# ArchDD/CPP-Raytracer-Rasterizer

Measured on AMD Instinct MI355X. Metric: Mrays/s (primary+shadow), higher is better.
Workload: dtype f32

## Files before the change

cpp-raytracer-rasterizer_amd/csrc/rt_trace.hip:

```cpp
#include "rt_trace_frame.hpp"

#include <float.h>

namespace mirt {


__global__ __launch_bounds__(256) void k_geo_table(const float *__restrict__ tris15, int n, GeoRow *__restrict__ geo, ShadeRow *__restrict__ shade)
{
    const int t = blockIdx.x * blockDim.x + threadIdx.x;
    if (t >= n) return;
    const float *t15 = tris15 + (size_t)15 * t;
    const v3 v0 = ld3(t15), e1 = sub3(ld3(t15 + 3), v0), e2 = sub3(ld3(t15 + 6), v0);
    GeoRow g;
    g.g0 = make_float4(v0.x, v0.y, v0.z, e1.x);
    g.g1 = make_float4(e1.y, e1.z, e2.x, e2.y);
    g.g2 = make_float4(e2.z, 0.0f, 0.0f, 0.0f);
    geo[t] = g;
    const v3 nd = normalize3(ld3(t15 + 9));
    ShadeRow sr;
    sr.n = make_float4(nd.x, nd.y, nd.z, 0.0f);
    sr.col = make_float4(t15[12], t15[13], t15[14], 0.0f);
    shade[t] = sr;
}

__global__ __launch_bounds__(256) void k_expand_light_rows(const uint32_t *__restrict__ bin_off, const uint32_t *__restrict__ entries,
                                                           int nlights, uint32_t keys_per_light,
                                                           const OriginRow *__restrict__ light_tab, int n,
                                                           LightRow *__restrict__ rows, const uint32_t *__restrict__ pair_count, uint32_t pair_cap,
                                                           uint32_t *__restrict__ row_tri )
{
    if (pair_count && *pair_count > pair_cap) return;
    const uint32_t first = bin_off[0], total = bin_off[(size_t)nlights * keys_per_light];
    for (uint32_t p = first + blockIdx.x * blockDim.x + threadIdx.x; p < total; p += gridDim.x * blockDim.x) {
        int k = 0;
        while (k + 1 < nlights && bin_off[(size_t)(k + 1) * keys_per_light] <= p) k++;
        const uint32_t tri = entries[p];
        rows[p] = light_tab[(size_t)k * n + tri];
        if (row_tri) row_tri[p] = tri;
    }
}

#ifndef MIRT_TR_STAGE
#define MIRT_TR_STAGE 16
#endif
constexpr int TR_STAGE = MIRT_TR_STAGE;
constexpr int TR_DRAIN = 64;
constexpr int TR_QUEUE = 96;
constexpr int TR_PIX = 128;
static_assert(TR_STAGE == 16, "the staging lanes are split 16 / 16 between the two tiles");

struct TrWaveLds {
    union {
        struct {
            float4 rows[TR_STAGE * 6];
            float4 geo[TR_STAGE * 2 * 3];
        };
        struct {
            float4 ray[TR_PIX];
            uint8_t sink;
        };
    };
    float4 q[TR_QUEUE];
    unsigned long long best[TR_PIX];
    uint2 qa[TR_QUEUE];
    union {
        float px[TR_PIX];
        float thr[TR_PIX];
    };
    float py[TR_PIX], pz[TR_PIX];
    uint8_t flag[TR_PIX];
};
static_assert(sizeof(TrWaveLds) % 16 == 0, "per-wave LDS slice must keep 16-byte alignment");
static_assert(sizeof(TrWaveLds) == 8064, "20 waves share a CU's LDS: the ray table overlays the staging, it adds nothing");

__device__ __forceinline__ void wave_lds_fence()
{
    __builtin_amdgcn_fence(__ATOMIC_RELEASE, "wavefront");
    __builtin_amdgcn_wave_barrier();
    __builtin_amdgcn_fence(__ATOMIC_ACQUIRE, "wavefront");
}

template <bool SHADOW>
__device__ __forceinline__ void tr_drain(TrWaveLds &s, int lane, int count, const float4 *__restrict__ geo, v3 start,
                                         const uint32_t *__restrict__ row_tri = nullptr, bool lazy_geo = false)
{
    wave_lds_fence();
    if (lane < count) {
        const float4 e = s.q[lane];
        uint2 a = s.qa[lane];
        float t, u, v;
        div3_sel(e.w, e.y, e.z, e.x, __builtin_amdgcn_ballot_w64(exact_quotients_outside(e.w, e.y, e.z, e.x)), t, u, v);
        if (u + v <= 1.0f && u >= 0.0f && v >= 0.0f && t >= 0.0f) {
            float4 g0, g1, g2;
            if (SHADOW) {
                const uint32_t tri = row_tri ? row_tri[a.y] : a.y;
                const float4 *g = geo + (size_t)tri * 3;
                g0 = g[0]; g1 = g[1]; g2 = g[2];
            } else if (lazy_geo) {
                const float4 *g = geo + (size_t)a.y * 3;
                g0 = g[0]; g1 = g[1]; g2 = g[2];
                a.x &= 0xFFu;
            } else {
                const float4 *g = s.geo + (a.x >> 8) * 3;
                g0 = g[0]; g1 = g[1]; g2 = g[2];
                a.x &= 0xFFu;
            }
            const v3 v0 = V3(g0.x, g0.y, g0.z), e1 = V3(g0.w, g1.x, g1.y), e2 = V3(g1.z, g1.w, g2.x);
            const v3 p = add3(add3(v0, scale3(e1, u)), scale3(e2, v));
            const float dist = distance3(start, p);
            if (SHADOW) {
                if (dist < s.thr[a.x]) s.flag[a.x] = 1;
            } else {
                s.flag[a.x] = 1;
                const unsigned long long key = min_t_key(dist, (int)a.y);
                atomicMin(&s.best[a.x], key);
                __builtin_amdgcn_fence(__ATOMIC_ACQ_REL, "wavefront");
                if (s.best[a.x] == key) { s.px[a.x] = p.x; s.py[a.x] = p.y; s.pz[a.x] = p.z; }
            }
        }
    }
    wave_lds_fence();
}

template <bool SHADOW>
__device__ __forceinline__ void tr_drain_full(TrWaveLds &s, int lane, int &qn, const float4 *__restrict__ geo, v3 start,
                                              const uint32_t *__restrict__ row_tri = nullptr, bool lazy_geo = false)
{
    tr_drain<SHADOW>(s, lane, TR_DRAIN, geo, start, row_tri, lazy_geo);
    const int rest = qn - TR_DRAIN;
    float4 e = make_float4(0.0f, 0.0f, 0.0f, 0.0f);
    uint2 a = make_uint2(0u, 0u);
    if (lane < rest) { e = s.q[TR_DRAIN + lane]; a = s.qa[TR_DRAIN + lane]; }
    wave_lds_fence();
    if (lane < rest) { s.q[lane] = e; s.qa[lane] = a; }
    qn = rest;
    wave_lds_fence();
}

__device__ __forceinline__ unsigned long long wballot(bool p) { return __builtin_amdgcn_ballot_w64(p); }

__device__ __forceinline__ int wave_rank(unsigned long long m)
{
    return (int)__builtin_amdgcn_mbcnt_hi((uint32_t)(m >> 32), __builtin_amdgcn_mbcnt_lo((uint32_t)m, 0u));
}

__device__ __forceinline__ void cube_bin_of2(const v3p &rd, uint32_t face_base0, int cube_bins, uint32_t *bin0, uint32_t *bin1)
{
    f2 a, b, m;
    int face[2];
#pragma unroll
    for (int h = 0; h < 2; h++) {
        const float x = h ? rd.x.y : rd.x.x, y = h ? rd.y.y : rd.y.x, z = h ? rd.z.y : rd.z.x;
        const float ax = fabsf(x), ay = fabsf(y), az = fabsf(z);
        int k;
        float mm, aa, bb, sgn;
        if (ax >= ay && ax >= az) { k = 0; mm = ax; sgn = x; aa = y; bb = z; }
        else if (ay >= az) { k = 1; mm = ay; sgn = y; aa = z; bb = x; }
        else { k = 2; mm = az; sgn = z; aa = x; bb = y; }
        face[h] = 2 * k + (sgn < 0.0f ? 1 : 0);
        if (h) { a.y = aa; b.y = bb; m.y = mm; } else { a.x = aa; b.x = bb; m.x = mm; }
    }
    const f2 im = { __builtin_amdgcn_rcpf(m.x), __builtin_amdgcn_rcpf(m.y) };
    const f2 u = a * im, v = b * im;
    const float half = 0.5f * (float)cube_bins;
    const uint32_t per_face = (uint32_t)(cube_bins * cube_bins);
#pragma unroll
    for (int h = 0; h < 2; h++) {
        const float uu = h ? u.y : u.x, vv = h ? v.y : v.x;
        int i = (int)floorf((uu + 1.0f) * half);
        int j = (int)floorf((vv + 1.0f) * half);
        i = min(max(i, 0), cube_bins - 1);
        j = min(max(j, 0), cube_bins - 1);
        const uint32_t bin = face_base0 + (uint32_t)face[h] * per_face + (uint32_t)j * cube_bins + (uint32_t)i;
        if (h) *bin1 = bin; else *bin0 = bin;
    }
}

__device__ __forceinline__ uint32_t cube_bin_of1(v3 rd, uint32_t face_base0, int cube_bins)
{
    const float ax = fabsf(rd.x), ay = fabsf(rd.y), az = fabsf(rd.z);
    int k;
    float m, a, b, sgn;
    if (ax >= ay && ax >= az) { k = 0; m = ax; sgn = rd.x; a = rd.y; b = rd.z; }
    else if (ay >= az) { k = 1; m = ay; sgn = rd.y; a = rd.z; b = rd.x; }
    else { k = 2; m = az; sgn = rd.z; a = rd.x; b = rd.y; }
    const int face = 2 * k + (sgn < 0.0f ? 1 : 0);
    const float im = __builtin_amdgcn_rcpf(m);
    const float u = a * im, v = b * im, half = 0.5f * (float)cube_bins;
    int i = (int)floorf((u + 1.0f) * half);
    int j = (int)floorf((v + 1.0f) * half);
    i = min(max(i, 0), cube_bins - 1);
    j = min(max(j, 0), cube_bins - 1);
    return face_base0 + (uint32_t)face * (uint32_t)(cube_bins * cube_bins) + (uint32_t)j * cube_bins + (uint32_t)i;
}


__global__ __launch_bounds__(64) void k_tile_order(const uint32_t *__restrict__ cam_off, int cam_shells, int tiles_x, int j0, int j1,
                                                   uint32_t *__restrict__ counters, uint32_t pair_cap, TilePairRec *__restrict__ order, uint32_t seg)
{
    const int pairs_x = (tiles_x + 1) / 2, lane = threadIdx.x;
    const int ty = j0 + (int)blockIdx.y, px = (int)blockIdx.x * 64 + lane;
    const uint32_t group = ((uint32_t)ty >> ORDER_STRIPE_SHIFT) & (ORDER_GROUPS - 1);
    TilePairRec r = { 0u, 0u, 0u, 0u };
    int cls = -1;
    if (px < pairs_x) {
        const uint32_t tile = (uint32_t)(ty * tiles_x + 2 * px);
        r.txy = (uint32_t)(2 * px) | ((uint32_t)ty << 16);
        cls = 0;
        if (counters[0] <= pair_cap) {
            const uint32_t b0 = cam_off[(size_t)tile * cam_shells], b1 = cam_off[(size_t)(tile + 1) * cam_shells];
            r.beg = b0; r.nA = b1 - b0;
            r.nB = 2 * px + 1 < tiles_x ? cam_off[(size_t)(tile + 2) * cam_shells] - b1 : 0u;
            cls = (int)min(max(r.nA, r.nB) / ORDER_CLASS_STEP, (uint32_t)(ORDER_CLASSES - 1));
        }
    }
    unsigned long long m[ORDER_CLASSES];
    uint32_t mine = 0;
#pragma unroll
    for (int c = 0; c < ORDER_CLASSES; c++) {
        m[c] = __builtin_amdgcn_ballot_w64(cls == c);
        if (lane == c) mine = (uint32_t)__popcll(m[c]);
    }
    uint32_t base = 0;
    if (lane < ORDER_CLASSES && mine) base = atomicAdd(&counters[16 + group * ORDER_CLASSES + lane], mine);
#pragma unroll
    for (int c = 0; c < ORDER_CLASSES; c++) {
        const uint32_t bc = (uint32_t)__builtin_amdgcn_readlane((int)base, c);
        if (cls == c) order[((size_t)group * ORDER_CLASSES + c) * seg + bc + (uint32_t)__popcll(m[c] & ((1ull << lane) - 1ull))] = r;
    }
}

#ifndef MIRT_TR_WAVES
#define MIRT_TR_WAVES 4
#endif
#ifndef MIRT_TR_WAVES_MIN
#define MIRT_TR_WAVES_MIN 3
#endif
template <bool AA, bool STATS, int WAVES = MIRT_TR_WAVES>
__global__ __launch_bounds__(64 * TR_WG_WAVES) __attribute__((amdgpu_waves_per_eu(WAVES == 5 ? 5 : MIRT_TR_WAVES_MIN, WAVES))) void k_rt_trace2(const RtTraceFrame tf)
{
    extern __shared__ __attribute__((aligned(16))) float4 s_all[];
    const RtFrame &f = tf.f;
    static_assert(TR_WG_WAVES == 1, "the wave -> tile pair map below and the LDS slice assume one wave per workgroup");
    const int lane = threadIdx.x & 63;
    TrWaveLds &s = reinterpret_cast<TrWaveLds *>(s_all)[0];

    const uint32_t group = blockIdx.x & (ORDER_GROUPS - 1);
    const uint32_t w = blockIdx.x >> 3;
    const uint32_t flags = tf.flags;
    const uint4 *cp = reinterpret_cast<const uint4 *>(__builtin_assume_aligned(tf.order_count + group * ORDER_CLASSES, 32));
    const uint4 c0 = cp[0], c1 = cp[1];
    const uint32_t npairs = *tf.pair_count, nlpairs = *tf.light_pair_count, nsel = *tf.sel_count;
    const int W = f.W, H = f.H;
    TilePairRec rec;
    {
        const uint32_t cnt[ORDER_CLASSES] = { c0.x, c0.y, c0.z, c0.w, c1.x, c1.y, c1.z, c1.w };
        uint32_t sum = 0, first = 0;
        int cls = ORDER_CLASSES - 1;
#pragma unroll
        for (int c = ORDER_CLASSES - 1; c >= 0; c--) {
            sum += cnt[c];
            const bool past = w >= sum;
            first = past ? sum : first;
            cls = past ? c - 1 : cls;
        }
        if (cls < 0) return;
        const uint32_t at = w - first;
        const uint4 r4 = *reinterpret_cast<const uint4 *>(tf.order + ((size_t)group * ORDER_CLASSES + (uint32_t)cls) * tf.order_seg + at);
        rec.txy = r4.x; rec.beg = r4.y; rec.nA = r4.z; rec.nB = r4.w;
    }
    const int txA = (int)(rec.txy & 0xFFFFu), ty = (int)(rec.txy >> 16);
    const bool enB = txA + 1 < tf.tiles_x;
    const int xA = txA * BIN_TILE + (lane & 7), xB = xA + BIN_TILE, y = ty * BIN_TILE + (lane >> 3);
    const bool okY = y >= f.y0 && y < f.y1;
    const bool okA = okY && xA < W, okB = enB && okY && xB < W;
    const unsigned long long okmA = wballot(okA), okmB = wballot(okB);
    const unsigned nokA = (unsigned)__popcll(okmA), nokB = (unsigned)__popcll(okmB);
#ifdef MIRT_TR_TIMING
    const long long tm0 = __builtin_amdgcn_s_memtime();
    long long tm_last = tm0, tm_seg[10] = { 0, 0, 0, 0, 0, 0, 0, 0, 0, 0 };
#define TM_SEG(i) { const long long now_ = __builtin_amdgcn_s_memtime(); tm_seg[i] += now_ - tm_last; tm_last = now_; }
#else
#define TM_SEG(i)
#endif
    const bool brute = npairs > tf.pair_cap;
    const bool brute_l = nlpairs > tf.light_pair_cap;
    const v3 cam = ld3(f.cam);
    const int rs = AA ? f.aa : 1;

    const uint32_t begA = rec.beg, begB = rec.beg + rec.nA;
    const uint32_t nall = brute ? min(nsel, (uint32_t)f.n) : 0u;
    const uint32_t nA = brute ? nall : rec.nA, nB = brute ? (enB ? nall : 0u) : rec.nB;
    const float4 *geo4 = reinterpret_cast<const float4 *>(tf.geo);
    const bool lazy = (flags & TRF_LAZY_GEO) != 0u;
    const bool list_end = (flags & TRF_LIST_END) != 0u && !brute;
    TM_SEG(0)

    float bdA = FLT_MAX, bdB = FLT_MAX;
    int biA = -1, biB = -1;
    v3 posA = V3(0.0f, 0.0f, 0.0f), posB = posA;
    v3p avg = splat3(V3(0.0f, 0.0f, 0.0f));
    unsigned ntests = 0, ncand = 0, nsteps_p = 0, nsteps_s = 0, ndrains = 0;
    unsigned ncand_l = 0;
    int qn = 0;
    const float hw = (float)W / 2.0f, hh = (float)H / 2.0f;

    f2 y1 = splat2(aa_start(y, rs));
    for (int z = 0; z < rs; z++) {
        f2 x1 = { aa_start(xA, rs), aa_start(xB, rs) };
        for (int z2 = 0; z2 < rs; z2++) {
            const v3p d = V3P(x1 - splat2(hw), y1 - splat2(hh), splat2(f.focal));
            const v3p nd = neg3p(mat3_mul_vecp(f.rot, d));

            s.best[lane] = MIN_T_NONE; s.best[lane + 64] = MIN_T_NONE;
            s.flag[lane] = 0; s.flag[lane + 64] = 0;
            float lbA = okA ? FLT_MAX : -__builtin_huge_valf(), lbB = okB ? FLT_MAX : -__builtin_huge_valf();
            float tbA = FLT_MAX, tbB = FLT_MAX;
            uint32_t liveA = nA, liveB = nB;
            for (uint32_t base = 0; base < max(liveA, liveB); base += TR_STAGE) {
                const int cntA = (int)min((uint32_t)TR_STAGE, liveA > base ? liveA - base : 0u);
                const int cntB = (int)min((uint32_t)TR_STAGE, liveB > base ? liveB - base : 0u);
                if (STATS) ncand += nokA * (unsigned)cntA + nokB * (unsigned)cntB;
                wave_lds_fence();
                float my_near = 0.0f;
                const int sh = lane >> 4, sj = lane & 15;
                const bool stage = lane < 32 && sj < (sh ? cntB : cntA);
                if (stage) {
                    const uint32_t idx = brute ? tf.sel[base + (uint32_t)sj] : tf.cam_entries[(sh ? begB : begA) + base + (uint32_t)sj];
                    const float4 *src = reinterpret_cast<const float4 *>(f.cam_tab + idx);
                    const float4 a0 = src[0], a1 = src[1], a2 = src[2];
                    if (!lazy) {
                        const float4 *gsrc = geo4 + (size_t)idx * 3;
                        float4 *gdst = s.geo + lane * 3;
                        gdst[0] = gsrc[0]; gdst[1] = gsrc[1]; gdst[2] = gsrc[2];
                    }
                    float *dst = reinterpret_cast<float *>(s.rows) + sj * 24 + sh;
                    dst[0] = a0.x; dst[2] = a0.y; dst[4] = a0.z; dst[6] = a0.w;
                    dst[8] = a1.x; dst[10] = a1.y; dst[12] = a1.z; dst[14] = a1.w;
                    dst[16] = a2.x; dst[18] = a2.y; dst[20] = a2.z; dst[22] = __uint_as_float(idx);
                    my_near = a1.w;
                } else if (lane < 32) {
                    reinterpret_cast<float *>(s.rows)[sj * 24 + sh + 14] = __builtin_huge_valf();
                }
                wave_lds_fence();
                TM_SEG(1)
                uint32_t pmA = (uint32_t)wballot(stage && sh == 0 && !(my_near > tbA)) & 0xFFFFu;
                uint32_t pmB = (uint32_t)(wballot(stage && sh == 1 && !(my_near > tbB)) >> 16) & 0xFFFFu;
                uint32_t pm = pmA | pmB;
                while (pm) {
                    const int j = __builtin_ctz(pm);
                    pm &= pm - 1u;
                    if (STATS) nsteps_p++;
                    const float4 *R = s.rows + 6 * j;
                    const float4 R0 = R[0], R1 = R[1], R2 = R[2], R3 = R[3], R4 = R[4], R5 = R[5];
                    TestDots2 td;
                    td.den = (f2){ R0.x, R0.y } * nd.x + (f2){ R0.z, R0.w } * nd.y + (f2){ R1.x, R1.y } * nd.z;
                    td.pu = (f2){ R2.x, R2.y } * nd.x + (f2){ R2.z, R2.w } * nd.y + (f2){ R3.x, R3.y } * nd.z;
                    td.qv = (f2){ R4.x, R4.y } * nd.x + (f2){ R4.z, R4.w } * nd.y + (f2){ R5.x, R5.y } * nd.z;
                    const f2 fm = maybe_hit2_margin(td);
                    const unsigned long long nearA = wballot(!(R3.z > lbA)), nearB = wballot(!(R3.w > lbB));
                    const unsigned long long filtA = wballot(fm.x >= MAYBE_HIT_THRESHOLD), filtB = wballot(fm.y >= MAYBE_HIT_THRESHOLD);
                    const unsigned long long mA = nearA & filtA, mB = nearB & filtB;
                    const bool passA0 = (mA >> lane) & 1ull, passB = (mB >> lane) & 1ull;
                    if (STATS) ntests += (unsigned)__popcll(nearA) + (unsigned)__popcll(nearB);
                    if (mA | mB) {
                        int cA = __popcll(mA);
                        const int cB = __popcll(mB);
                        bool passA = passA0;
                        if (qn + cA + cB > TR_QUEUE) {
                            TM_SEG(2)
                            if (qn) { tr_drain<false>(s, lane, qn, geo4, cam, nullptr, lazy); qn = 0; if (STATS) ndrains++; }
                            if (cA + cB > TR_QUEUE) {
                                if (passA) {
                                    const int at = wave_rank(mA);
                                    s.q[at] = make_float4(td.den.x, td.pu.x, td.qv.x, R1.z);
                                    s.qa[at] = make_uint2((uint32_t)lane | ((uint32_t)j << 8), __float_as_uint(R5.z));
                                }
                                tr_drain<false>(s, lane, cA, geo4, cam, nullptr, lazy); if (STATS) ndrains++;
                                passA = false; cA = 0;
                            }
                            TM_SEG(3)
                        }
                        if (passA) {
                            const int at = qn + wave_rank(mA);
                            s.q[at] = make_float4(td.den.x, td.pu.x, td.qv.x, R1.z);
                            s.qa[at] = make_uint2((uint32_t)lane | ((uint32_t)j << 8), __float_as_uint(R5.z));
                        }
                        if (passB) {
                            const int at = qn + cA + wave_rank(mB);
                            s.q[at] = make_float4(td.den.y, td.pu.y, td.qv.y, R1.w);
                            s.qa[at] = make_uint2(((uint32_t)lane + 64u) | ((uint32_t)(16 + j) << 8), __float_as_uint(R5.w));
                        }
                        qn += cA + cB;
                        if (qn >= TR_DRAIN) {
                            TM_SEG(2)
                            do { tr_drain_full<false>(s, lane, qn, geo4, cam, nullptr, lazy); if (STATS) ndrains++; } while (qn >= TR_DRAIN);
                            TM_SEG(3)
                            lbA = okA ? min_t_dist(s.best[lane]) : lbA; lbB = okB ? min_t_dist(s.best[lane + 64]) : lbB;
                            tbA = wave_max_f(lbA); tbB = wave_max_f(lbB);
                            pmA &= (uint32_t)wballot(stage && sh == 0 && !(my_near > tbA));
                            pmB &= (uint32_t)(wballot(stage && sh == 1 && !(my_near > tbB)) >> 16);
                            pm &= pmA | pmB;
                        }
                    }
                }
                TM_SEG(2)
                const bool more = base + TR_STAGE < max(liveA, liveB);
                if (qn) {
                    tr_drain<false>(s, lane, qn, geo4, cam, nullptr, lazy); qn = 0; if (STATS) ndrains++;
                    if (more) {
                        lbA = okA ? min_t_dist(s.best[lane]) : lbA; lbB = okB ? min_t_dist(s.best[lane + 64]) : lbB;
                        tbA = wave_max_f(lbA); tbB = wave_max_f(lbB);
                    }
                }
                if (more && list_end) {
                    const bool later = stage && bin_shell_of(my_near, tf.shell_d0, tf.shell_iw, tf.cam_shells) >
                                                bin_shell_of(sh ? tbB : tbA, tf.shell_d0, tf.shell_iw, tf.cam_shells);
                    const uint32_t lm = (uint32_t)wballot(later);
                    if (lm & 0xFFFFu) liveA = min(liveA, base + (uint32_t)TR_STAGE);
                    if (lm >> 16) liveB = min(liveB, base + (uint32_t)TR_STAGE);
                }
                TM_SEG(3)
            }
            const unsigned long long keyA = s.best[lane], keyB = s.best[lane + 64];
            const bool anyA = s.flag[lane] != 0, anyB = s.flag[lane + 64] != 0;
            if constexpr (AA) {
                if (anyA && bdA >= min_t_dist(keyA)) {
                    bdA = min_t_dist(keyA); biA = min_t_index(keyA);
                    posA = V3(s.px[lane], s.py[lane], s.pz[lane]);
                }
                if (anyB && bdB >= min_t_dist(keyB)) {
                    bdB = min_t_dist(keyB); biB = min_t_index(keyB);
                    posB = V3(s.px[lane + 64], s.py[lane + 64], s.pz[lane + 64]);
                }
            } else {
                const v3 hpA = V3(s.px[lane], s.py[lane], s.pz[lane]);
                const v3 hpB = V3(s.px[lane + 64], s.py[lane + 64], s.pz[lane + 64]);
                const bool takeA = anyA && bdA >= min_t_dist(keyA), takeB = anyB && bdB >= min_t_dist(keyB);
                bdA = takeA ? min_t_dist(keyA) : bdA; biA = takeA ? min_t_index(keyA) : biA;
                posA = V3(takeA ? hpA.x : posA.x, takeA ? hpA.y : posA.y, takeA ? hpA.z : posA.z);
                bdB = takeB ? min_t_dist(keyB) : bdB; biB = takeB ? min_t_index(keyB) : biB;
                posB = V3(takeB ? hpB.x : posB.x, takeB ? hpB.y : posB.y, takeB ? hpB.z : posB.z);
            }

            TM_SEG(4)
            const bool hitA = okA && anyA, hitB = okB && anyB;
            const unsigned long long hmA = wballot(hitA), hmB = wballot(hitB);
            const unsigned nhits = (unsigned)(__popcll(hmA) + __popcll(hmB));
            if (hmA | hmB) {
                const ShadeRow *srA = tf.shade + (biA >= 0 ? biA : 0), *srB = tf.shade + (biB >= 0 ? biB : 0);
                const float4 nA4 = srA->n, nB4 = srB->n;
                float4 cA4 = make_float4(0.0f, 0.0f, 0.0f, 0.0f), cB4 = cA4;
                if constexpr (WAVES != 5) { cA4 = srA->col; cB4 = srB->col; }
                const v3p pos = join3(posA, posB);
                const v3p nDir = join3(V3(nA4.x, nA4.y, nA4.z), V3(nB4.x, nB4.y, nB4.z));
                v3p result = splat3(V3(0.0f, 0.0f, 0.0f)), result2 = result;
                const bool one_sample = (flags & TRF_ONE_SAMPLE) != 0u;
                int samples_left = one_sample ? 1 : f.samples;
                for (int k = 0; k < f.nlights; k++) {
                    const v3 L = ld3(f.lpos[k]);
                    const LightGeometry2 lg = light_geometry2(pos, L, ld3(f.lcol[k]), f.lights_in_range != 0, hitA, hitB);
                    const f2 r = lg.r;
                    const v3p rd = lg.rDir, B = lg.B;
                    const f2 dn = dot3p(rd, nDir);
                    const f2 mx = { (dn.x < 0.0f) ? 0.0f : dn.x, (dn.y < 0.0f) ? 0.0f : dn.y };
                    v3p D = scale3p(B, mx);
                    const f2 thr = r * splat2(0.99f);
                    const bool needA = hitA && shadow_ray_needed(D.x.x, D.y.x, D.z.x), needB = hitB && shadow_ray_needed(D.x.y, D.y.y, D.z.y);
                    const unsigned long long nmA = wballot(needA), nmB = wballot(needB);
                    const int nrA = __popcll(nmA), nrays = nrA + __popcll(nmB);
                    TM_SEG(5)
                    if (nrays) {
                        wave_lds_fence();
                        s.thr[lane] = thr.x; s.thr[lane + 64] = thr.y;
                        s.flag[lane] = 0; s.flag[lane + 64] = 0;
                        if (needA) s.ray[wave_rank(nmA)] = make_float4(rd.x.x, rd.y.x, rd.z.x, __uint_as_float((uint32_t)lane));
                        if (needB) s.ray[nrA + wave_rank(nmB)] = make_float4(rd.x.y, rd.y.y, rd.z.y, __uint_as_float((uint32_t)lane + 64u));
                        wave_lds_fence();
                        const bool two = nrays > 64;
                        const bool has0 = lane < nrays, has1 = lane + 64 < nrays;
                        const float4 ry0 = s.ray[has0 ? lane : 0];
                        float4 ry1 = ry0;
                        if (two) ry1 = s.ray[has1 ? lane + 64 : 0];
                        const v3 rd0 = V3(ry0.x, ry0.y, ry0.z), rd1 = V3(ry1.x, ry1.y, ry1.z);
                        const uint32_t pix0 = __float_as_uint(ry0.w), pix1 = __float_as_uint(ry1.w);
                        const float thr0 = s.thr[pix0], thr1 = s.thr[pix1];
                        uint32_t e0 = 0, end0 = 0, e1 = 0, end1 = 0;
                        const float4 *rows4;
                        if (brute_l) {
                            rows4 = reinterpret_cast<const float4 *>(f.light_tab + (size_t)k * f.n);
                            if (has0) end0 = (uint32_t)f.n;
                            if (has1) end1 = (uint32_t)f.n;
                        } else {
                            rows4 = reinterpret_cast<const float4 *>(tf.light_rows);
                            const uint32_t face0 = (uint32_t)k * 6u * (uint32_t)(tf.cube_bins * tf.cube_bins);
                            const BinFrameDesc *lf = tf.light_frames + 6 * k;
                            const int ns = tf.light_shells;
                            const float sd0 = lf->shell_d0, siw = lf->shell_iw;
                            if (two) {
                                uint32_t bin0, bin1;
                                cube_bin_of2(join3(rd0, rd1), face0, tf.cube_bins, &bin0, &bin1);
                                const uint32_t sh0 = bin_shell_of(thr0, sd0, siw, ns), sh1 = bin_shell_of(thr1, sd0, siw, ns);
                                const uint32_t key0 = bin0 * (uint32_t)ns, key1 = bin1 * (uint32_t)ns;
                                const uint32_t o00 = tf.light_off[key0], o01 = tf.light_off[key0 + sh0 + 1u];
                                const uint32_t o10 = tf.light_off[key1], o11 = tf.light_off[key1 + sh1 + 1u];
                                e0 = o00; end0 = o01;
                                e1 = has1 ? o10 : 0u; end1 = has1 ? o11 : 0u;
                            } else {
                                const uint32_t key0 = cube_bin_of1(rd0, face0, tf.cube_bins) * (uint32_t)ns;
                                const uint32_t sh0 = bin_shell_of(thr0, sd0, siw, ns);
                                const uint32_t o00 = tf.light_off[key0], o01 = tf.light_off[key0 + sh0 + 1u];
                                e0 = has0 ? o00 : 0u; end0 = has0 ? o01 : 0u;
                            }
                        }
                        if (STATS) ncand_l += (end0 - e0) + (end1 - e1);
                        const uint32_t *row_tri = brute_l ? nullptr : tf.light_tri;
                        const bool first0 = e0 < end0;
                        uint32_t e = first0 ? e0 : e1, end = first0 ? end0 : end1, pix = first0 ? pix0 : pix1;
                        v3 crd = V3(first0 ? rd0.x : rd1.x, first0 ? rd0.y : rd1.y, first0 ? rd0.z : rd1.z);
                        float cthr = first0 ? thr0 : thr1;
                        end1 = first0 ? end1 : 0u;
                        float4 c0, c1, c2;
                        { const float4 *src = rows4 + (size_t)(e < end ? e : 0u) * 3; c0 = src[0]; c1 = src[1]; c2 = src[2]; }
                        TM_SEG(6)
                        const int not_brute = brute_l ? 0 : 1;
                        for (;;) {
                            const bool act = e < end;
                            const unsigned long long am = wballot(act);
                            if (!am) break;
                            if (STATS) { nsteps_s++; ntests += (unsigned)__popcll(am); }
                            const TestDots td = test_dots(c0, c1, c2, crd);
                            const int pass = (int)act & (int)!(c1.w > cthr) & (int)maybe_hit(td);
                            const int sure = pass & not_brute & (int)(c2.w < cthr) & (int)sure_hit(td, c0.w);
                            const int queue = pass & (sure ^ 1);
                            const unsigned long long m = wballot(queue != 0);
                            int done = sure;
                            *(sure ? &s.flag[pix] : &s.sink) = 1;
                            if (m) {
                                if (qn + __popcll(m) > TR_QUEUE) { tr_drain<true>(s, lane, qn, geo4, L, row_tri); qn = 0; if (STATS) ndrains++; }
                                if (queue) {
                                    const int at = qn + wave_rank(m);
                                    s.q[at] = make_float4(td.den, td.pu, td.qv, c0.w);
                                    s.qa[at] = make_uint2(pix, e);
                                }
                                qn += __popcll(m);
                                if (qn >= TR_DRAIN) {
                                    TM_SEG(7)
                                    do { tr_drain_full<true>(s, lane, qn, geo4, L, row_tri); if (STATS) ndrains++; } while (qn >= TR_DRAIN);
                                    TM_SEG(8)
                                    done |= (int)act & (int)(s.flag[pix] != 0);
                                }
                            }
                            const int cont = (int)act & (done ^ 1) & (int)(e + 1u < end);
                            const int sw = (int)act & (cont ^ 1) & (int)(e1 < end1);
                            crd = V3(sw ? rd1.x : crd.x, sw ? rd1.y : crd.y, sw ? rd1.z : crd.z);
                            cthr = sw ? thr1 : cthr;
                            pix = sw ? pix1 : pix;
                            e = cont ? e + 1u : (sw ? e1 : end);
                            end = sw ? end1 : end;
                            end1 = sw ? 0u : end1;
                            const float4 *src = rows4 + (size_t)((cont | sw) ? e : 0u) * 3;
                            c0 = src[0]; c1 = src[1]; c2 = src[2];
                        }
                        TM_SEG(7)
                        if (qn) { tr_drain<true>(s, lane, qn, geo4, L, row_tri); qn = 0; if (STATS) ndrains++; }
                        TM_SEG(8)
                        wave_lds_fence();
                        if (s.flag[lane] != 0) { D.x.x = 0.0f; D.y.x = 0.0f; D.z.x = 0.0f; }
                        if (s.flag[lane + 64] != 0) { D.x.y = 0.0f; D.y.y = 0.0f; D.z.y = 0.0f; }
                    }
                    result = add3p(result, D);
                    if (one_sample || --samples_left == 0) {
                        result2 = add3p(result2, result);
                        samples_left = f.samples;
                    }
                }
                if constexpr (WAVES == 5) { cA4 = srA->col; cB4 = srB->col; }
                const v3p tcol = join3(V3(cA4.x, cA4.y, cA4.z), V3(cB4.x, cB4.y, cB4.z));
                const v3p Dl = mul3p(result2, tcol);
                const v3p shaded = add3p(avg, mul3p(tcol, add3p(Dl, splat3(ld3(f.indirect)))));
                avg = join3(hitA ? half0(shaded) : half0(avg), hitB ? half1(shaded) : half1(avg));
                if (AA) x1 = x1 + (f2){ hitA ? aa_step(rs) : 0.0f, hitB ? aa_step(rs) : 0.0f };
            }
            if (lane == 0 && nhits) {
                const unsigned shard = blockIdx.x % HIT_SHARDS;
                atomicAdd(f.hit_count + (size_t)shard * HIT_SHARD_STRIDE, (unsigned long long)nhits);
            }
            wave_lds_fence();
        }
        if (AA) y1 = y1 + splat2(aa_step(rs));
    }
    {
        if (STATS) ncand += wave_sum(ncand_l);
        const unsigned shard = blockIdx.x % HIT_SHARDS;
#ifdef MIRT_TR_TIMING
#ifndef MIRT_TR_TIMING_FIRST
#define MIRT_TR_TIMING_FIRST 0
#endif
        TM_SEG(9)
        if (lane == 0) {
            for (int i = 0; i < 10; i++) atomicAdd(f.hit_count + (size_t)shard * HIT_SHARD_STRIDE + 3 + (i + 10 - MIRT_TR_TIMING_FIRST) % 10, (unsigned long long)tm_seg[i]);
            atomicMax(f.hit_count + (size_t)shard * HIT_SHARD_STRIDE + 13, (unsigned long long)(tm_last - tm0));
        }
        const unsigned v = lane == 0 ? ntests : ncand;
        if (lane < 2 && v) atomicAdd(f.hit_count + (size_t)shard * HIT_SHARD_STRIDE + 1 + lane, (unsigned long long)v);
#else
        const unsigned v = lane == 0 ? ntests : lane == 1 ? ncand : lane == 2 ? nsteps_p : lane == 3 ? nsteps_s : ndrains;
        if (STATS && lane < 5 && v) atomicAdd(f.hit_count + (size_t)shard * HIT_SHARD_STRIDE + 1 + lane, (unsigned long long)v);
#endif
    }
    if (AA) {
        const f2 q = splat2((float)(rs * rs));
        avg = V3P(div2(avg.x, q), div2(avg.y, q), div2(avg.z, q));
    }
    {
        uint32_t *const xrgb = f.xrgb;
        const size_t xrow = (size_t)(y - f.row_origin) * f.pitch_words;
        const bool inY = y >= 1 && y < H - 1;
        const int xlast = W - 1;
        if (flags & TRF_PLANES) {
            float *const rgb = f.rgb, *const fd = f.fd, *const dist = f.dist, *const pos = f.pos;
            int32_t *const index = f.index;
            const float focal_plane = f.focal_plane;
            const size_t row = (size_t)y * W;
            if (okA) {
                const size_t px = row + xA;
                if (rgb) st3(rgb + 3 * px, half0(avg));
                if (index) index[px] = biA;
                if (fd) fd[px] = biA >= 0 ? bdA - focal_plane : 0.0f;
                if (dist) dist[px] = biA >= 0 ? bdA : 3.402823466e+38f;
                if (pos) st3(pos + 3 * px, biA >= 0 ? posA : V3(0.0f, 0.0f, 0.0f));
            }
            if (okB) {
                const size_t px = row + xB;
                if (rgb) st3(rgb + 3 * px, half1(avg));
                if (index) index[px] = biB;
                if (fd) fd[px] = biB >= 0 ? bdB - focal_plane : 0.0f;
                if (dist) dist[px] = biB >= 0 ? bdB : 3.402823466e+38f;
                if (pos) st3(pos + 3 * px, biB >= 0 ? posB : V3(0.0f, 0.0f, 0.0f));
            }
        }
        if (okA && inY && xA >= 1 && xA < xlast) xrgb[xrow + xA] = pack_xrgb(half0(avg));
        if (okB && inY && xB >= 1 && xB < xlast) xrgb[xrow + xB] = pack_xrgb(half1(avg));
    }
}

template __global__ void k_rt_trace2<false, false>(const RtTraceFrame);
template __global__ void k_rt_trace2<false, false, 5>(const RtTraceFrame);
template __global__ void k_rt_trace2<false, true>(const RtTraceFrame);
template __global__ void k_rt_trace2<true, false>(const RtTraceFrame);
template __global__ void k_rt_trace2<true, true>(const RtTraceFrame);

size_t rt_trace_lds_bytes(int waves) { return (size_t)waves * sizeof(TrWaveLds); }

}
```

Baseline: 57270.

## Software-prefetch next stage of candidate triangle rows into registers

Moves the index-list and cam_tab/geo row loads for each staging step one iteration ahead. The next stage's rows are fetched into registers right after the current stage is written to LDS, so global-load latency overlaps the intersection loop. The per-stage body then only copies registers to LDS. It also adds an explicit s_waitcnt in the lazy-geo hit path and a compiler barrier in the LDS path to control scheduling. The cost is higher register pressure from the prefetched float4s, which may reduce occupancy.

```diff
diff --git a/cpp-raytracer-rasterizer_amd/csrc/rt_trace.hip b/cpp-raytracer-rasterizer_amd/csrc/rt_trace.hip
--- a/cpp-raytracer-rasterizer_amd/csrc/rt_trace.hip
+++ b/cpp-raytracer-rasterizer_amd/csrc/rt_trace.hip
@@ -100,10 +100,12 @@
                 const float4 *g = geo + (size_t)a.y * 3;
                 g0 = g[0]; g1 = g[1]; g2 = g[2];
                 a.x &= 0xFFu;
+                __builtin_amdgcn_s_waitcnt(0x0F70);
             } else {
                 const float4 *g = s.geo + (a.x >> 8) * 3;
                 g0 = g[0]; g1 = g[1]; g2 = g[2];
                 a.x &= 0xFFu;
+                asm volatile("" ::: "memory");
             }
             const v3 v0 = V3(g0.x, g0.y, g0.z), e1 = V3(g0.w, g1.x, g1.y), e2 = V3(g1.z, g1.w, g2.x);
             const v3 p = add3(add3(v0, scale3(e1, u)), scale3(e2, v));
@@ -271,6 +273,37 @@
     }
     const int txA = (int)(rec.txy & 0xFFFFu), ty = (int)(rec.txy >> 16);
     const bool enB = txA + 1 < tf.tiles_x;
+    const bool brute = npairs > tf.pair_cap;
+    const uint32_t begA = rec.beg, begB = rec.beg + rec.nA;
+    const uint32_t nall = brute ? min(nsel, (uint32_t)f.n) : 0u;
+    const uint32_t nA = brute ? nall : rec.nA, nB = brute ? (enB ? nall : 0u) : rec.nB;
+    const float4 *geo4 = reinterpret_cast<const float4 *>(tf.geo);
+    const bool lazy = (flags & TRF_LAZY_GEO) != 0u;
+    const int sh = (lane >> 4) & 1, sj = lane & 15;
+    const uint32_t *const lst = brute ? tf.sel : tf.cam_entries + (sh ? begB : begA);
+    const uint32_t nmine = sh ? nB : nA;
+    uint32_t pidx, nidx;
+    float4 pa0, pa1, pa2, pg0, pg1, pg2;
+    auto fetch_rows = [&]() {
+        const float4 *src = reinterpret_cast<const float4 *>(f.cam_tab + pidx);
+        pa0 = src[0]; pa1 = src[1]; pa2 = src[2];
+        if (!lazy) {
+            const float4 *gsrc = geo4 + (size_t)pidx * 3;
+            pg0 = gsrc[0]; pg1 = gsrc[1]; pg2 = gsrc[2];
+        }
+    };
+    auto fetch_first = [&]() {
+        if constexpr (AA) {
+            pidx = nidx = 0u;
+            pa0 = pa1 = pa2 = pg0 = pg1 = pg2 = make_float4(0.0f, 0.0f, 0.0f, 0.0f);
+        }
+        if (lane < 32) {
+            if ((uint32_t)sj < nmine) pidx = lst[sj];
+            if ((uint32_t)(sj + TR_STAGE) < nmine) nidx = lst[sj + TR_STAGE];
+            if ((uint32_t)sj < nmine) fetch_rows();
+        }
+    };
+    if constexpr (!AA) fetch_first();
     const int xA = txA * BIN_TILE + (lane & 7), xB = xA + BIN_TILE, y = ty * BIN_TILE + (lane >> 3);
     const bool okY = y >= f.y0 && y < f.y1;
     const bool okA = okY && xA < W, okB = enB && okY && xB < W;
@@ -283,16 +316,10 @@
 #else
 #define TM_SEG(i)
 #endif
-    const bool brute = npairs > tf.pair_cap;
     const bool brute_l = nlpairs > tf.light_pair_cap;
     const v3 cam = ld3(f.cam);
     const int rs = AA ? f.aa : 1;
 
-    const uint32_t begA = rec.beg, begB = rec.beg + rec.nA;
-    const uint32_t nall = brute ? min(nsel, (uint32_t)f.n) : 0u;
-    const uint32_t nA = brute ? nall : rec.nA, nB = brute ? (enB ? nall : 0u) : rec.nB;
-    const float4 *geo4 = reinterpret_cast<const float4 *>(tf.geo);
-    const bool lazy = (flags & TRF_LAZY_GEO) != 0u;
     const bool list_end = (flags & TRF_LIST_END) != 0u && !brute;
     TM_SEG(0)
 
@@ -309,6 +336,7 @@
     for (int z = 0; z < rs; z++) {
         f2 x1 = { aa_start(xA, rs), aa_start(xB, rs) };
         for (int z2 = 0; z2 < rs; z2++) {
+            if constexpr (AA) fetch_first();
             const v3p d = V3P(x1 - splat2(hw), y1 - splat2(hh), splat2(f.focal));
             const v3p nd = neg3p(mat3_mul_vecp(f.rot, d));
 
@@ -323,26 +351,28 @@
                 if (STATS) ncand += nokA * (unsigned)cntA + nokB * (unsigned)cntB;
                 wave_lds_fence();
                 float my_near = 0.0f;
-                const int sh = lane >> 4, sj = lane & 15;
                 const bool stage = lane < 32 && sj < (sh ? cntB : cntA);
                 if (stage) {
-                    const uint32_t idx = brute ? tf.sel[base + (uint32_t)sj] : tf.cam_entries[(sh ? begB : begA) + base + (uint32_t)sj];
-                    const float4 *src = reinterpret_cast<const float4 *>(f.cam_tab + idx);
-                    const float4 a0 = src[0], a1 = src[1], a2 = src[2];
                     if (!lazy) {
-                        const float4 *gsrc = geo4 + (size_t)idx * 3;
                         float4 *gdst = s.geo + lane * 3;
-                        gdst[0] = gsrc[0]; gdst[1] = gsrc[1]; gdst[2] = gsrc[2];
+                        gdst[0] = pg0; gdst[1] = pg1; gdst[2] = pg2;
                     }
                     float *dst = reinterpret_cast<float *>(s.rows) + sj * 24 + sh;
-                    dst[0] = a0.x; dst[2] = a0.y; dst[4] = a0.z; dst[6] = a0.w;
-                    dst[8] = a1.x; dst[10] = a1.y; dst[12] = a1.z; dst[14] = a1.w;
-                    dst[16] = a2.x; dst[18] = a2.y; dst[20] = a2.z; dst[22] = __uint_as_float(idx);
-                    my_near = a1.w;
+                    dst[0] = pa0.x; dst[2] = pa0.y; dst[4] = pa0.z; dst[6] = pa0.w;
+                    dst[8] = pa1.x; dst[10] = pa1.y; dst[12] = pa1.z; dst[14] = pa1.w;
+                    dst[16] = pa2.x; dst[18] = pa2.y; dst[20] = pa2.z; dst[22] = __uint_as_float(pidx);
+                    my_near = pa1.w;
                 } else if (lane < 32) {
                     reinterpret_cast<float *>(s.rows)[sj * 24 + sh + 14] = __builtin_huge_valf();
                 }
                 wave_lds_fence();
+                if (base + TR_STAGE < max(liveA, liveB)) {
+                    const uint32_t live = sh ? liveB : liveA, at = base + (uint32_t)(TR_STAGE + sj);
+                    if (lane < 32) {
+                        if (at < live) { pidx = nidx; fetch_rows(); }
+                        if (at + TR_STAGE < live) nidx = lst[at + TR_STAGE];
+                    }
+                }
                 TM_SEG(1)
                 uint32_t pmA = (uint32_t)wballot(stage && sh == 0 && !(my_near > tbA)) & 0xFFFFu;
                 uint32_t pmB = (uint32_t)(wballot(stage && sh == 1 && !(my_near > tbB)) >> 16) & 0xFFFFu;
```

After: 57690 (median of 6 runs). About the same (+0.7%).
